# shininglegend/cs420-ray-tracer

Hardware: NVIDIA B200
Metric: Mrays/s (higher is better)
Workload: dtype f32 filter / f64 decide

## Files before the change

cs420-ray-tracer_b200/csrc/exact_fp64.cuh:

```cuda
#ifndef RT_EXACT_FP64_CUH
#define RT_EXACT_FP64_CUH

#include <cuda_runtime.h>

namespace rtx {

struct d3 { double x, y, z; };

#define RT_DF __device__ __forceinline__

RT_DF double dadd(double a, double b) { return __dadd_rn(a, b); }
RT_DF double dsub(double a, double b) { return __dsub_rn(a, b); }
RT_DF double dmul(double a, double b) { return __dmul_rn(a, b); }
RT_DF double ddiv(double a, double b) { return __ddiv_rn(a, b); }
RT_DF double dsqrt(double a) { return __dsqrt_rn(a); }

RT_DF d3 mk(double x, double y, double z) { d3 r; r.x = x; r.y = y; r.z = z; return r; }
RT_DF d3 add(d3 a, d3 b) { return mk(dadd(a.x, b.x), dadd(a.y, b.y), dadd(a.z, b.z)); }
RT_DF d3 sub(d3 a, d3 b) { return mk(dsub(a.x, b.x), dsub(a.y, b.y), dsub(a.z, b.z)); }
RT_DF d3 scale(d3 a, double t) { return mk(dmul(a.x, t), dmul(a.y, t), dmul(a.z, t)); }
RT_DF double dot(d3 a, d3 b) { return dadd(dadd(dmul(a.x, b.x), dmul(a.y, b.y)), dmul(a.z, b.z)); }
RT_DF double length(d3 a) { return dsqrt(dot(a, a)); }
RT_DF d3 normalized(d3 a) { double len = length(a); return mk(ddiv(a.x, len), ddiv(a.y, len), ddiv(a.z, len)); }

RT_DF double std_max(double a, double b) { return (a < b) ? b : a; }
RT_DF double std_min(double a, double b) { return (b < a) ? b : a; }

RT_DF bool intersect(d3 o, d3 d, double a, d3 c, double r2, double &t) {
  d3 oc = sub(o, c);
  double b = dmul(2.0, dot(oc, d));
  double cc = dsub(dot(oc, oc), r2);
  double disc = dsub(dmul(b, b), dmul(dmul(4.0, a), cc));
  if (disc < 0) return false;
  double two_a = dmul(2.0, a);
  if (disc == 0) { t = ddiv(-b, two_a); return true; }
  double s = dsqrt(disc);
  double t1 = ddiv(dsub(-b, s), two_a);
  double t2 = ddiv(dadd(-b, s), two_a);
  if (std_max(t1, t2) < 0) return false;
  t = std_min(t1, t2);
  if (t < 0) t = std_max(t1, t2);
  return true;
}

RT_DF d3 hit_point(d3 o, d3 d, double t) { return add(o, scale(d, t)); }
RT_DF d3 normal_at(d3 p, d3 c) { return normalized(sub(p, c)); }

RT_DF void reflect_ray(d3 d, d3 hit, d3 n, double eps, d3 &o2, d3 &d2) {
  d3 rd = sub(d, scale(scale(n, 2.0), dot(d, n)));
  o2 = add(hit, scale(n, eps));
  d2 = normalized(rd);
}

RT_DF void shadow_ray(d3 p, d3 lpos, double eps, d3 &o2, d3 &d2, double &ldist) {
  d3 to_light = sub(lpos, p);
  ldist = length(to_light);
  d3 ldir = normalized(to_light);
  o2 = add(p, scale(ldir, eps));
  d2 = normalized(ldir);
}

RT_DF d3 camera_dir(d3 fwd, d3 right, d3 up, double su, double sv) {
  d3 dir = add(add(fwd, scale(right, su)), scale(up, sv));
  return normalized(normalized(dir));
}

}
#endif
```

Baseline: 18610.

## Replace fp64 divides with reciprocal-FMA path and skip redundant renormalization

Normalization now computes one reciprocal of the length and uses an FMA-corrected multiply per component, with a guarded exponent-range check that falls back to true division. Re-normalizing an already unit vector uses a cheap near-one test that often returns the vector unchanged. Sphere intersection also skips computing the second root when the first is already non-negative. The aim is to cut expensive fp64 divide and sqrt sequences on a GPU with limited fp64 throughput, at the cost of relying on correct-rounding arguments that must match the reference bit for bit.

```diff
diff --git a/cs420-ray-tracer_b200/csrc/exact_fp64.cuh b/cs420-ray-tracer_b200/csrc/exact_fp64.cuh
--- a/cs420-ray-tracer_b200/csrc/exact_fp64.cuh
+++ b/cs420-ray-tracer_b200/csrc/exact_fp64.cuh
@@ -21,7 +21,34 @@
 RT_DF d3 scale(d3 a, double t) { return mk(dmul(a.x, t), dmul(a.y, t), dmul(a.z, t)); }
 RT_DF double dot(d3 a, d3 b) { return dadd(dadd(dmul(a.x, b.x), dmul(a.y, b.y)), dmul(a.z, b.z)); }
 RT_DF double length(d3 a) { return dsqrt(dot(a, a)); }
-RT_DF d3 normalized(d3 a) { double len = length(a); return mk(ddiv(a.x, len), ddiv(a.y, len), ddiv(a.z, len)); }
+
+RT_DF unsigned exp_off(double v) { return (((unsigned)__double2hiint(v) >> 20) & 0x7ffu) - 768u; }
+RT_DF bool div_ok(unsigned ex_off_or) { return ex_off_or < 512u; }
+RT_DF double recip(double b) { return __drcp_rn(b); }
+RT_DF double div_core(double x, double b, double y) {
+  const double q = dmul(x, y);
+  const double r = __fma_rn(-b, q, x);
+  return __fma_rn(r, y, q);
+}
+__device__ __noinline__ d3 div3_slow(d3 a, double len) { return mk(ddiv(a.x, len), ddiv(a.y, len), ddiv(a.z, len)); }
+RT_DF d3 div3_by(d3 a, double len, double rl) {
+  if (div_ok(exp_off(a.x) | exp_off(a.y) | exp_off(a.z) | exp_off(len)))
+    return mk(div_core(a.x, len, rl), div_core(a.y, len, rl), div_core(a.z, len, rl));
+  return div3_slow(a, len);
+}
+RT_DF d3 normalized(d3 a) { const double len = length(a); return div3_by(a, len, recip(len)); }
+__device__ __noinline__ d3 normalized_call(d3 a) { return normalized(a); }
+
+RT_DF d3 renormalized(d3 u) {
+  const double s = dot(u, u);
+  const double d = dsub(s, 1.0);
+  if (fabs(d) < 0x1p-47) {
+    const double len = __fma_rd(d, 0.5, 1.0);
+    if (len == 1.0) return u;
+    return div3_by(u, len, __dsub_ru(2.0, len));
+  }
+  return normalized_call(u);
+}
 
 RT_DF double std_max(double a, double b) { return (a < b) ? b : a; }
 RT_DF double std_min(double a, double b) { return (b < a) ? b : a; }
@@ -36,6 +63,7 @@
   if (disc == 0) { t = ddiv(-b, two_a); return true; }
   double s = dsqrt(disc);
   double t1 = ddiv(dsub(-b, s), two_a);
+  if (!(t1 < 0) && two_a > 0) { t = t1; return true; }
   double t2 = ddiv(dadd(-b, s), two_a);
   if (std_max(t1, t2) < 0) return false;
   t = std_min(t1, t2);
@@ -57,12 +85,12 @@
   ldist = length(to_light);
   d3 ldir = normalized(to_light);
   o2 = add(p, scale(ldir, eps));
-  d2 = normalized(ldir);
+  d2 = renormalized(ldir);
 }
 
 RT_DF d3 camera_dir(d3 fwd, d3 right, d3 up, double su, double sv) {
   d3 dir = add(add(fwd, scale(right, su)), scale(up, sv));
-  return normalized(normalized(dir));
+  return renormalized(normalized(dir));
 }
 
 }
```

Result: faster. 19040 (median of 6 runs) (+2.3%).
